# fims9000/SYNT_ISIC

Measured on AMD Instinct MI355X. Metric: images/sec at 3x64x64 T=1000 (DDPM reverse-diffusion sampling), higher is better.
Workload: dtype f32

## Files before the change

synt_isic_amd/csrc/common.h:

```cpp
#pragma once

#include <hip/hip_runtime.h>

#include <atomic>
#include <cstdarg>
#include <cstdint>
#include <cstdio>
#include <string>
#include <map>
#include <mutex>
#include <vector>

#include "../../include/sisic.h"

namespace sisic {

void set_error(const char* fmt, ...);

#define SISIC_HIP(call)                                                                   \
    do {                                                                                  \
        hipError_t _e = (call);                                                           \
        if (_e != hipSuccess) {                                                           \
            ::sisic::set_error("%s failed: %s (%s:%d)", #call, hipGetErrorString(_e),     \
                               __FILE__, __LINE__);                                       \
            return SISIC_EHIP;                                                            \
        }                                                                                 \
    } while (0)

#define SISIC_REQUIRE(cond, ...)                 \
    do {                                         \
        if (!(cond)) {                           \
            ::sisic::set_error(__VA_ARGS__);     \
            return SISIC_EINVAL;                 \
        }                                        \
    } while (0)

#define SISIC_TRY(expr)             \
    do {                            \
        int _rc = (expr);           \
        if (_rc != SISIC_OK) return _rc; \
    } while (0)

enum ProfileKind { PK_CONV3 = 0, PK_CONV1 = 1, PK_GN = 2, PK_ATTN = 3, PK_DDPM = 4, PK_OTHER = 5, PK_WINO_MAIN = 6, PK_WINO_BF3 = 7, PK_COUNT = 8 };

struct ProfileSlot {
    double ms = 0, bytes = 0, flops = 0, flops_exec = 0;
    int64_t launches = 0;
};

struct PendingEvent {
    hipEvent_t start, stop;
    int kind;
    int kind2;
};

}

struct sisic_ctx {
    int device = 0;
    int num_cus = 0;
    bool profiling = false;
    sisic::ProfileSlot prof[sisic::PK_COUNT];
    std::vector<sisic::PendingEvent> pending;
    std::vector<hipEvent_t> event_pool;
    struct SplitK { float* p = nullptr; size_t floats = 0; };
    std::map<hipStream_t, SplitK> splitk;
    std::mutex splitk_mutex;
    std::atomic<uint64_t> scratch_generation{0};
};

namespace sisic {

struct ProfileScope {
    sisic_ctx* ctx;
    hipStream_t stream;
    PendingEvent ev{};
    bool active = false;
    ProfileScope(sisic_ctx* c, hipStream_t s, int kind, double bytes, double flops, double flops_exec = -1.0, int kind2 = -1);
    ~ProfileScope();
};

int profile_collect(sisic_ctx* ctx);

inline int ensure_dynamic_lds(sisic_ctx* ctx, const void* kern, int bytes, std::atomic<uint64_t>& done) {
    const uint64_t bit = uint64_t(1) << (ctx->device & 63);
    if (done.load(std::memory_order_acquire) & bit) return SISIC_OK;
    SISIC_HIP(hipFuncSetAttribute(kern, hipFuncAttributeMaxDynamicSharedMemorySize, bytes));
    done.fetch_or(bit, std::memory_order_release);
    return SISIC_OK;
}

inline int cdiv(int a, int b) { return (a + b - 1) / b; }
inline int wino_latency_ksplit(int Cout, int Cin, int Hout, int Wout) {
    const int co_t = Cout > 64 ? 128 : 64;
    const int per_image = cdiv(Hout, 8) * cdiv(Wout, 16) * cdiv(Cout, co_t);
    const int nchunks = cdiv(Cin, 8);
    int k = 1;
    while (per_image * k < 256 && k < 8 && nchunks % (2 * k) == 0) k *= 2;
    return k;
}
inline int wino_latency_segments(int Hout, int Wout) { return cdiv(Hout * Wout, 1024); }
inline int64_t cdiv64(int64_t a, int64_t b) { return (a + b - 1) / b; }
inline int round_up(int a, int b) { return cdiv(a, b) * b; }

constexpr int CONV_CO_TILE = 64;
inline int conv_ci_chunk(int ksize) { return ksize == 1 ? 32 : (ksize == 3 ? 16 : 4); }
inline int conv_cin_pad(int cin, int ksize) { return round_up(cin, conv_ci_chunk(ksize)); }
inline int conv_cout_pad(int cout) { return round_up(cout, CONV_CO_TILE); }
inline int64_t conv_packed_floats(int cout, int cin, int ksize) {
    const int64_t first = (int64_t)conv_cin_pad(cin, ksize) * ksize * ksize * conv_cout_pad(cout);
    return ksize == 1 ? 3 * first + first / 2 : first;
}

int launch_conv2d(sisic_ctx*, const sisic_conv_args& a, hipStream_t s);
int launch_conv_smallcout(sisic_ctx*, const sisic_conv_args& a, hipStream_t s);
int launch_score_head_bwd(sisic_ctx*, const float* logits, const float* fc_w, const float* act, float* g, int B, int C,
                          int HW, int n_classes, int target, hipStream_t s);
int launch_relu_bwd(sisic_ctx*, const float* dy, const float* y, float* out, int64_t n, hipStream_t s);
int launch_scatter_add_even(sisic_ctx*, float* dst, const float* src, int planes, int H, int W, hipStream_t s);
int launch_maxpool_bwd(sisic_ctx*, const float* dm, const float* xin, float* dx, int planes, int H, int W, hipStream_t s);
int launch_stem_bwd(sisic_ctx*, const float* g, const float* w_oihw, float* dp, int B, int CO, int OH, int OW, int H, int W,
                    hipStream_t s);
int launch_preprocess_bwd(sisic_ctx*, const float* dp, const float* x, float* dx, int B, int H, int W, int OH, int OW,
                          hipStream_t s);
int launch_add_relu(sisic_ctx*, const float* y, const float* identity, float* out, int64_t n, hipStream_t s);
int launch_gradcam(sisic_ctx*, const float* y, const float* outp, const float* fc_w, const float* bias, float* cam, int B, int C,
                   int h, int w, int S, int target, hipStream_t s);
int conv_stats_slots(const sisic_conv_args& a);
bool conv_finalizes(const sisic_conv_args& a);
bool conv_pointwise_applicable(const sisic_conv_args& a);
int conv_pointwise_stats_slots(const sisic_conv_args& a);
int launch_conv_pointwise(sisic_ctx*, const sisic_conv_args& a, hipStream_t s);
bool conv_pointwise_bf3_applicable(const sisic_conv_args& a);
int launch_conv_pointwise_bf3(sisic_ctx*, const sisic_conv_args& a, hipStream_t s);
int launch_gn_finalize(sisic_ctx*, const float* st0, int c0, int slots0, const float* st1, int c1, int slots1, int B,
                       int HW, int groups, float eps, const float* gamma, const float* beta, float* scale, float* shift,
                       hipStream_t s, float* mean_rstd = nullptr);
int launch_conv_winograd(sisic_ctx*, const sisic_conv_args& a, const float* u_packed, int cfg, hipStream_t s);
int launch_winograd_pack(sisic_ctx*, const float* w, int Cout, int Cin, float* packed, hipStream_t s);
int64_t winograd_packed_numel(int Cout, int Cin);
inline int64_t winograd_first_floats(int Cout, int Cin) { return (int64_t)round_up(Cin, 16) * 16 * conv_cout_pad(Cout); }
int launch_conv_pack(sisic_ctx*, const float* w, int Cout, int Cin, int k, float* packed, hipStream_t s);
int launch_gn_stats(sisic_ctx*, const float* in0, int c0, const float* in1, int c1, int B, int HW, int groups,
                    float eps, const float* gamma, const float* beta, float* scale, float* shift, hipStream_t s,
                    float* mean_rstd = nullptr);
int launch_attention(sisic_ctx*, const float* qkv, float* out, int B, int C, int N, int head_dim, hipStream_t s);
int launch_ddpm_step(sisic_ctx*, const float* eps, const float* x, const float* z, float* out, int64_t n,
                     float sb, float sa, float c0, float c1, float sigma, float clip, hipStream_t s);
size_t loop_state_bytes();
int launch_loop_select_row(sisic_ctx*, const float* table, int R, const void* state, float* out, hipStream_t s);
int launch_loop_advance(sisic_ctx*, void* state, hipStream_t s);
int launch_ddpm_step_indexed(sisic_ctx*, const float* eps, float* x, int64_t n, const void* state, const float* coef,
                             const int* zrow, float clip, hipStream_t s);
int launch_denorm_u8(sisic_ctx*, const float* x, uint8_t* out, int B, int C, int H, int W, hipStream_t s, int form = 0);
int launch_temb_mlp(sisic_ctx*, const float* t_vals, int B, const float* freqs, int n_freqs, const float* w1t,
                    const float* b1, const float* w2t, const float* b2, int hidden, float* temb_act, hipStream_t s,
                    float* save_emb = nullptr, float* save_h1 = nullptr, float* save_t2 = nullptr);
int launch_linear_t(sisic_ctx*, const float* x, int B, int K, const float* wt, const float* bias, int R,
                    float* out, hipStream_t s);
int launch_transpose2d(sisic_ctx*, const float* in, int rows, int cols, float* out, int out_ld, int out_col0,
                       hipStream_t s);
int launch_preprocess(sisic_ctx*, const float* x, float* out, int B, int H, int W, int OH, int OW, hipStream_t s);
int launch_maxpool(sisic_ctx*, const float* x, float* out, int B, int C, int H, int W, hipStream_t s);
int launch_avgpool_fc(sisic_ctx*, const float* x, const float* w, const float* bias, float* out, int B, int C, int HW,
                      int n_out, hipStream_t s);
int launch_class_scores(sisic_ctx*, const float* logits, int B, int n, int target, float* prob, float* logscore,
                        hipStream_t s);
int launch_mask_patches(sisic_ctx*, const float* image, const uint8_t* masks, float* out, int S, int C, int H, int W,
                        int patch, hipStream_t s);

}
```

synt_isic_amd/csrc/conv_mfma.hip:

```cpp
#include <cstdlib>
#include <type_traits>

#include "common.h"
#include "pack_device.h"

namespace sisic {

typedef float f32x16 __attribute__((ext_vector_type(16)));

struct ConvParams {
    const float* in0;
    const float* in1;
    int c0, c1;
    int B, Hin, Win;
    int Hc, Wc;
    int Hout, Wout;
    int ups;
    int zero_insert;
    const float* w;
    int cout_pad;
    const float* bias;
    int Cout;
    const float* gn_scale;
    const float* gn_shift;
// ... 108 lines not shown
    const int a_base = half * G::KK * G::CO_TILE + wm * MT * 32 + l31;
    int b_base;
    {
        const int pix = wn * NT * 32 + l31;
        const int y = pix / TW, x = pix % TW;
        b_base = half * G::CHS + (y * STRIDE) * G::IW + x * STRIDE;
    }
    constexpr int NT_STEP = (TW >= 32) ? ((TW > 32) ? 32 * STRIDE : STRIDE * G::IW) : (32 / TW) * STRIDE * G::IW;
    static_assert(TW >= 32 || 32 % TW == 0, "TW must divide 32");
    static_assert(TW <= 32 || TW % 32 == 0, "TW must be a multiple of 32");

    f32x16 acc[MT][NT];
#pragma unroll
    for (int m = 0; m < MT; ++m)
#pragma unroll
        for (int n = 0; n < NT; ++n)
#pragma unroll
            for (int r = 0; r < 16; ++r) acc[m][n][r] = 0.0f;

    float rin[G::EPT];
    float rw[G::W_F4_PT * 4];
    float gsc = 1.0f, gsh = 0.0f;
    bool cval = false;

    const int prologue = (p.gn_scale == nullptr) ? 0 : (p.gn_silu ? 2 : 1);

    auto load_chunk = [&](int chunk) __attribute__((always_inline)) {
        const int c = chunk * CIC + sci;
        cval = c < Cin;
        const int cc = min(c, Cin - 1);
        const float* src = (cc < p.c0) ? p.in0 + ((size_t)b * p.c0 + cc) * HWin
                                       : p.in1 + ((size_t)b * p.c1 + (cc - p.c0)) * HWin;
        if constexpr (V4) {
#pragma unroll
            for (int i = 0; i < EPT4; ++i) {
                const float4 t = *reinterpret_cast<const float4*>(src + goff4[i]);
                rin[4 * i + 0] = t.x; rin[4 * i + 1] = t.y; rin[4 * i + 2] = t.z; rin[4 * i + 3] = t.w;
            }
        } else {
#pragma unroll
            for (int i = 0; i < G::EPT; ++i) rin[i] = src[goff[i]];
        }
        if (prologue) {
            gsc = p.gn_scale[(size_t)b * Cin + cc];
            gsh = p.gn_shift[(size_t)b * Cin + cc];
        }
        const float* wsrc = p.w + (size_t)chunk * CIC * G::KK * p.cout_pad + co0;
#pragma unroll
        for (int i = 0; i < G::W_F4_PT; ++i) {
            const int f = min(tid + i * G::NTHR, G::W_F4 - 1);
            const int rr = f / (G::CO_TILE / 4), c4 = f % (G::CO_TILE / 4);
            const float4 t = *reinterpret_cast<const float4*>(wsrc + (size_t)rr * p.cout_pad + c4 * 4);
            rw[4 * i + 0] = t.x; rw[4 * i + 1] = t.y; rw[4 * i + 2] = t.z; rw[4 * i + 3] = t.w;
        }
    };

    auto store_chunk = [&](const int buf) __attribute__((always_inline)) {
        float* dst = in_lds + buf * G::IN_BUF + sci * G::CHS + sl;
        const unsigned m = cval ? vmask : 0u;
        float v[G::EPT];
        if (prologue == 2) {
#pragma unroll
            for (int i = 0; i < G::EPT; ++i) v[i] = silu_f(rin[i] * gsc + gsh);
        } else if (prologue == 1) {
#pragma unroll
            for (int i = 0; i < G::EPT; ++i) v[i] = rin[i] * gsc + gsh;
        } else {
#pragma unroll
            for (int i = 0; i < G::EPT; ++i) v[i] = rin[i];
        }
        if constexpr (V4) {
            float* dst4 = in_lds + buf * G::IN_BUF + sci * G::CHS + 4 * sl;
            const unsigned m4 = cval ? vmask4 : 0u;
#pragma unroll
            for (int i = 0; i < EPT4; ++i) {
                const bool on = (m4 >> i) & 1u;
                *reinterpret_cast<float4*>(dst4 + i * G::TPC * 4) =
                    make_float4(on ? v[4 * i + 0] : 0.0f, on ? v[4 * i + 1] : 0.0f, on ? v[4 * i + 2] : 0.0f, on ? v[4 * i + 3] : 0.0f);
            }
        } else {
#pragma unroll
            for (int i = 0; i < G::EPT; ++i) dst[i * G::TPC] = ((m >> i) & 1u) ? v[i] : 0.0f;
        }
        float* wdst = w_lds + buf * G::W_BUF + tid * 4;
#pragma unroll
        for (int i = 0; i < G::W_F4_PT; ++i)
            *reinterpret_cast<float4*>(wdst + i * G::NTHR * 4) =
                make_float4(rw[4 * i + 0], rw[4 * i + 1], rw[4 * i + 2], rw[4 * i + 3]);
    };

    auto compute_chunk = [&](const int buf) __attribute__((always_inline)) {
        const float* A = w_lds + buf * G::W_BUF + a_base;
        const float* Bm = in_lds + buf * G::IN_BUF + b_base;
#pragma unroll
        for (int cp = kg * (CIC / 2 / KSP); cp < (kg + 1) * (CIC / 2 / KSP); ++cp) {
#pragma unroll
            for (int ky = 0; ky < KS; ++ky) {
#pragma unroll
                for (int kx = 0; kx < KS; ++kx) {
                    float a[MT], bb[NT];
#pragma unroll
                    for (int m = 0; m < MT; ++m)
                        a[m] = A[(2 * cp * G::KK + ky * KS + kx) * G::CO_TILE + m * 32];
#pragma unroll
                    for (int n = 0; n < NT; ++n)
                        bb[n] = Bm[2 * cp * G::CHS + ky * G::IW + kx + n * NT_STEP];
#pragma unroll
                    for (int m = 0; m < MT; ++m)
#pragma unroll
                        for (int n = 0; n < NT; ++n)
                            acc[m][n] = __builtin_amdgcn_mfma_f32_32x32x2f32(a[m], bb[n], acc[m][n], 0, 0, 0);
                }
            }
        }
    };

    load_chunk(0);
    store_chunk(0);
    __syncthreads();
    auto step = [&](const int chunk, auto buf_tag) __attribute__((always_inline)) {
        constexpr int BUF = decltype(buf_tag)::value;
        const bool more = chunk + 1 < p.nchunks;
        if (more) load_chunk(chunk + 1);
        compute_chunk(BUF);
        if (more) store_chunk(BUF ^ 1);
        __syncthreads();
    };
    {
        int chunk = 0;
        for (; chunk + 1 < p.nchunks; chunk += 2) {
            step(chunk, std::integral_constant<int, 0>{});
            step(chunk + 1, std::integral_constant<int, 1>{});
        }
        if (chunk < p.nchunks) step(chunk, std::integral_constant<int, 0>{});
    }

    if constexpr (KSP > 1) {
        static_assert(KSP == 2, "two K groups");
        static_assert((size_t)WM * WN * MT * NT * 16 * 64 * sizeof(float) <= G::LDS_BYTES, "reduction slab fits the staging LDS");
        float* red = smem + (size_t)wq * MT * NT * 16 * 64 + lane;
        if (kg == 1) {
#pragma unroll
            for (int m = 0; m < MT; ++m)
#pragma unroll
                for (int n = 0; n < NT; ++n)
#pragma unroll
                    for (int r = 0; r < 16; ++r) red[((m * NT + n) * 16 + r) * 64] = acc[m][n][r];
        }
        __syncthreads();
        if (kg != 0) return;
#pragma unroll
        for (int m = 0; m < MT; ++m)
#pragma unroll
            for (int n = 0; n < NT; ++n)
#pragma unroll
                for (int r = 0; r < 16; ++r) acc[m][n][r] += red[((m * NT + n) * 16 + r) * 64];
    }

    const size_t HWout = (size_t)p.Hout * p.Wout;
    float cbias[MT][16];
#pragma unroll
    for (int m = 0; m < MT; ++m) {
#pragma unroll
        for (int r = 0; r < 16; ++r) {
            cbias[m][r] = 0.0f;
        }
    }
    if (p.bias) {
#pragma unroll
        for (int m = 0; m < MT; ++m)
#pragma unroll
            for (int r = 0; r < 16; ++r)
                cbias[m][r] += p.bias[min(co0 + wm * MT * 32 + m * 32 + (r & 3) + 8 * (r >> 2) + 4 * half, p.Cout - 1)];
    }
    if (p.chan_bias) {
        const float* cb = p.chan_bias + (size_t)b * p.chan_bias_stride;
#pragma unroll
        for (int m = 0; m < MT; ++m)
#pragma unroll
            for (int r = 0; r < 16; ++r)
                cbias[m][r] += cb[min(co0 + wm * MT * 32 + m * 32 + (r & 3) + 8 * (r >> 2) + 4 * half, p.Cout - 1)];
    }
    float psum[MT][16];
#pragma unroll
    for (int m = 0; m < MT; ++m)
#pragma unroll
        for (int r = 0; r < 16; ++r) psum[m][r] = 0.0f;
    unsigned pvmask = 0;
#pragma unroll
    for (int n = 0; n < NT; ++n) {
        const int pix = wn * NT * 32 + n * 32 + l31;
        const int oy = oy0 + pix / TW, ox = ox0 + pix % TW;
        const bool pv = oy < p.Hout && ox < p.Wout;
        pvmask |= pv ? (1u << n) : 0u;
        const size_t pix_off = (size_t)min(oy, p.Hout - 1) * p.Wout + min(ox, p.Wout - 1);
#pragma unroll
        for (int m = 0; m < MT; ++m) {
            float res[16];
#pragma unroll
            for (int r = 0; r < 16; ++r) res[r] = 0.0f;
            if (p.residual) {
#pragma unroll
                for (int r = 0; r < 16; ++r) {
                    const int co = min(co0 + wm * MT * 32 + m * 32 + (r & 3) + 8 * (r >> 2) + 4 * half, p.Cout - 1);
                    res[r] = p.residual[((size_t)b * p.Cout + co) * HWout + pix_off];
                }
            }
#pragma unroll
            for (int r = 0; r < 16; ++r) {
                const int co = co0 + wm * MT * 32 + m * 32 + (r & 3) + 8 * (r >> 2) + 4 * half;
                float v = acc[m][n][r] + cbias[m][r] + res[r];
                if (p.relu) v = fmaxf(v, 0.0f);
                if (pv && co < p.Cout) p.out[((size_t)b * p.Cout + co) * HWout + pix_off] = v;
                acc[m][n][r] = v;
                psum[m][r] += pv ? v : 0.0f;
            }
        }
    }

    if (p.stats) {
        const float cnt = half_wave_sum((float)__builtin_popcount(pvmask));
        const float inv = 1.0f / fmaxf(cnt, 1.0f);
        const int slots = p.tiles_x * p.tiles_y * WN, slot = (ty * p.tiles_x + tx) * WN + wn;
#pragma unroll
        for (int m = 0; m < MT; ++m) {
#pragma unroll
            for (int r = 0; r < 16; ++r) {
                const int co = co0 + wm * MT * 32 + m * 32 + (r & 3) + 8 * (r >> 2) + 4 * half;
                const float s1 = half_wave_sum(psum[m][r]);
                const float mean = s1 * inv;
                float q = 0.0f;
#pragma unroll
                for (int n = 0; n < NT; ++n) {
                    const float d = acc[m][n][r] - mean;
                    q += ((pvmask >> n) & 1u) ? d * d : 0.0f;
                }
                q = half_wave_sum(q);
                if (l31 == 0 && co < p.Cout)
                    reinterpret_cast<float4*>(p.stats)[((size_t)b * p.Cout + co) * slots + slot] = make_float4(cnt, s1, q, 0.0f);
            }
        }
    }
}


__global__ void conv_pack_kernel(const float* __restrict__ w, int Cout, int Cin, int KK, int cin_pad, int cout_pad,
                                 float* __restrict__ out) {
    const size_t first = (size_t)cin_pad * KK * cout_pad;
    const size_t total = KK == 1 ? 3 * first + first / 2 : first;
    for (size_t i = (size_t)blockIdx.x * blockDim.x + threadIdx.x; i < total; i += (size_t)gridDim.x * blockDim.x) {
        conv_pack_elem(i, w, Cout, Cin, KK, cin_pad, cout_pad, out);
    }
}

template <int KS, int STRIDE, int MT, int NT, int WM, int WN, int TW, int CIC, int OCC = 2, int KSP = 1>
static int launch_cfg(sisic_ctx* ctx, ConvParams& p, hipStream_t s) {
    using G = ConvGeom<KS, STRIDE, MT, NT, WM, WN, TW, CIC, KSP>;
    p.tiles_x = cdiv(p.Wout, TW);
    p.tiles_y = cdiv(p.Hout, G::TH);
    p.n_co_tiles = p.cout_pad / G::CO_TILE;
    p.nchunks = cdiv(p.c0 + p.c1, CIC);
    const int64_t nwg = (int64_t)p.B * p.tiles_x * p.tiles_y * p.n_co_tiles;
    SISIC_REQUIRE(nwg > 0 && nwg < (int64_t(1) << 31), "conv2d: grid of %lld workgroups unsupported", (long long)nwg);
    p.nwg = (int)nwg;
    if (p.slots_query) {
        *p.slots_query = p.tiles_x * p.tiles_y * WN;
        return SISIC_OK;
    }
    if constexpr (KS == 1 && STRIDE == 1 && TW == G::PIX && G::EPT % 4 == 0) {
        const bool aligned = ((reinterpret_cast<uintptr_t>(p.in0) | reinterpret_cast<uintptr_t>(p.in1)) & 15) == 0;
        if (p.Wc % 4 == 0 && aligned) {
            auto kern4 = conv_mfma_kernel<KS, STRIDE, MT, NT, WM, WN, TW, CIC, OCC, KSP, true>;
            static std::atomic<uint64_t> lds_opt_in4{0};
            SISIC_TRY(ensure_dynamic_lds(ctx, reinterpret_cast<const void*>(kern4), (int)G::LDS_BYTES, lds_opt_in4));
            hipLaunchKernelGGL(kern4, dim3(p.nwg), dim3(G::NTHR), G::LDS_BYTES, s, p);
            SISIC_HIP(hipGetLastError());
            return SISIC_OK;
        }
    }
    auto kern = conv_mfma_kernel<KS, STRIDE, MT, NT, WM, WN, TW, CIC, OCC, KSP>;
    static std::atomic<uint64_t> lds_opt_in{0};
    SISIC_TRY(ensure_dynamic_lds(ctx, reinterpret_cast<const void*>(kern), (int)G::LDS_BYTES, lds_opt_in));
    hipLaunchKernelGGL(kern, dim3(p.nwg), dim3(G::NTHR), G::LDS_BYTES, s, p);
    SISIC_HIP(hipGetLastError());
    return SISIC_OK;
}

int launch_conv_pack(sisic_ctx*, const float* w, int Cout, int Cin, int k, float* packed, hipStream_t s) {
    SISIC_REQUIRE(k == 1 || k == 3 || k == 7, "conv_pack: ksize %d unsupported", k);
    const int cin_pad = conv_cin_pad(Cin, k), cout_pad = conv_cout_pad(Cout);
    const size_t total = (size_t)cin_pad * k * k * cout_pad;
    const int blocks = (int)std::min<size_t>((total * (k == 1 ? 4 : 1) + 255) / 256, 4096);
    hipLaunchKernelGGL(conv_pack_kernel, dim3(blocks), dim3(256), 0, s, w, Cout, Cin, k * k, cin_pad, cout_pad, packed);
    SISIC_HIP(hipGetLastError());
    return SISIC_OK;
}

static int dispatch_conv2d(sisic_ctx* ctx, const sisic_conv_args& a, hipStream_t s, int* slots_query);

static int winograd_cfg(const sisic_conv_args& a) {
    if (!(a.ksize == 3 && a.stride == 1 && a.w_winograd != nullptr && a.Cout > 4) || a.upsample == 2) return 0;
    if ((a.tile_cfg >= 60 && a.tile_cfg <= 74) || a.tile_cfg == 78 || a.tile_cfg == 79 || (a.tile_cfg >= 90 && a.tile_cfg <= 92)) return a.tile_cfg;
    if (a.tile_cfg != 0) return 0;
    const int Hout = a.Hin << (a.upsample ? 1 : 0), Wout = a.Win << (a.upsample ? 1 : 0);
    const bool fits32 = 16.0 * std::max(a.c0, a.c1) * a.Hin * a.Win < 4294967296.0;
    if (!fits32) return 0;
    if (Hout >= 12 && Wout >= 12) {
        static const bool wide_on = [] { const char* e = std::getenv("SISIC_WINO_WIDE"); return !e || std::atoi(e) != 0; }();
        static const bool bf3_on = [] { const char* e = std::getenv("SISIC_WINO_BF16X3"); return !e || std::atoi(e) != 0; }();
        const int th = (Hout + 15) / 16 * 16, tw = (Wout + 15) / 16 * 16;
        if (bf3_on && a.Cout % 64 == 0 && 4 * Hout * Wout >= 3 * th * tw && a.c0 + a.c1 >= 16 &&
            a.c0 + a.c1 <= 2048 &&
            4.0 * a.Cout * Hout * Wout < 2147483648.0)
            return 74;
        if (wide_on && !a.upsample) return a.Cout > 64 ? 68 : 69;
        return 66;
    }
    const int Cin = a.c0 + a.c1;
    static const bool ksplit_on = [] { const char* e = std::getenv("SISIC_KSPLIT"); return !e || std::atoi(e) != 0; }();
    if (ksplit_on && Hout <= 8 && Wout <= 8 && Hout >= 5 && Wout >= 5 && Cin >= 128 && Cin % 32 == 0 && a.Cout >= 128) {
        static const bool wide_on = [] { const char* e = std::getenv("SISIC_WINO_WIDE"); return !e || std::atoi(e) != 0; }();
        static const bool bf3_on = [] { const char* e = std::getenv("SISIC_WINO_BF16X3"); return !e || std::atoi(e) != 0; }();
        if (bf3_on && !a.upsample && a.Cout % 64 == 0 && Cin <= 512) return 92;
        return (wide_on && !a.upsample) ? 91 : 90;
    }
    return 0;
}
static bool winograd_selected(const sisic_conv_args& a) { return winograd_cfg(a) != 0; }

int conv_stats_slots(const sisic_conv_args& a) {
    if (const int cfg = winograd_cfg(a)) {
        if (cfg >= 90 && cfg <= 92) return 1;
        const int Hout = a.Hin << (a.upsample ? 1 : 0), Wout = a.Win << (a.upsample ? 1 : 0);
        if ((cfg == 78 || cfg == 79) && wino_latency_ksplit(a.Cout, a.c0 + a.c1, Hout, Wout) > 1) return wino_latency_segments(Hout, Wout);
        if ((cfg >= 68 && cfg <= 73) || cfg == 78 || cfg == 79) return ((Hout + 7) / 8) * ((Wout + 15) / 16);
        const int edge = (cfg == 61 || cfg == 63 || cfg == 65 || cfg == 67) ? 8 : 16;
        return ((Hout + edge - 1) / edge) * ((Wout + edge - 1) / edge);
    }
    int slots = 0;
    sisic_conv_args q = a;
    q.stats_out = nullptr;
    if (dispatch_conv2d(nullptr, q, nullptr, &slots) != SISIC_OK) return 0;
    return slots;
}

bool conv_finalizes(const sisic_conv_args& a) {
    if (!a.fin_gamma || a.fin_groups <= 0) return false;
    const int cfg = winograd_cfg(a);
    const int Hout = a.Hin << (a.upsample ? 1 : 0), Wout = a.Win << (a.upsample ? 1 : 0);
    if (a.Cout % a.fin_groups != 0 || a.Cout / a.fin_groups != 8) return false;
    if (cfg == 74) return !a.upsample && Hout <= 16 && Wout <= 16 && a.Cout % 64 == 0;
    if (cfg < 90 || cfg > 92) return false;
    if (Hout * Wout != 64 || a.Cout % 16 != 0) return false;
    return ((reinterpret_cast<uintptr_t>(a.residual) | reinterpret_cast<uintptr_t>(a.out) | reinterpret_cast<uintptr_t>(a.stats_out)) & 15) == 0;
}

int launch_conv2d(sisic_ctx* ctx, const sisic_conv_args& a, hipStream_t s) { return dispatch_conv2d(ctx, a, s, nullptr); }

static int dispatch_conv2d(sisic_ctx* ctx, const sisic_conv_args& a, hipStream_t s, int* slots_query) {
    SISIC_REQUIRE(a.in0 && a.w_packed && a.out, "conv2d: null tensor");
    SISIC_REQUIRE(a.B > 0 && a.Hin > 0 && a.Win > 0 && a.c0 > 0 && a.c1 >= 0 && a.Cout > 0, "conv2d: bad shape");
    SISIC_REQUIRE((a.c1 == 0) == (a.in1 == nullptr), "conv2d: in1/c1 mismatch");
    SISIC_REQUIRE(a.ksize == 1 || a.ksize == 3 || a.ksize == 7, "conv2d: ksize %d unsupported", a.ksize);
    SISIC_REQUIRE(a.stride == 1 || a.stride == 2, "conv2d: stride %d unsupported", a.stride);
    SISIC_REQUIRE(a.ksize != 7 || a.stride == 2, "conv2d: 7x7 is built for stride 2 only (the ResNet stem)");
    SISIC_REQUIRE(!(a.upsample && a.stride != 1), "conv2d: upsample with stride");
    SISIC_REQUIRE((a.gn_scale == nullptr) == (a.gn_shift == nullptr), "conv2d: gn_scale/gn_shift mismatch");

    ConvParams p{};
    p.in0 = a.in0; p.in1 = a.in1; p.c0 = a.c0; p.c1 = a.c1;
    p.B = a.B; p.Hin = a.Hin; p.Win = a.Win;
    p.ups = a.upsample ? 1 : 0;
    p.zero_insert = a.upsample == 2 ? 1 : 0;
    p.Hc = a.Hin << p.ups; p.Wc = a.Win << p.ups;
    const int pad = a.ksize / 2;
    p.Hout = (p.Hc + 2 * pad - a.ksize) / a.stride + 1;
    p.Wout = (p.Wc + 2 * pad - a.ksize) / a.stride + 1;
    p.w = a.w_packed; p.cout_pad = conv_cout_pad(a.Cout);
    p.bias = a.bias; p.Cout = a.Cout;
    p.gn_scale = a.gn_scale; p.gn_shift = a.gn_shift; p.gn_silu = a.gn_silu;
    p.chan_bias = a.chan_bias; p.chan_bias_stride = a.chan_bias_stride; p.residual = a.residual; p.relu = a.relu; p.out = a.out;
    p.stats = a.stats_out; p.slots_query = slots_query;

    const int Cin = a.c0 + a.c1;
    const double kk = double(a.ksize) * a.ksize;
    const double out_elems = double(a.B) * a.Cout * p.Hout * p.Wout;
    const double bytes = 4.0 * (double(a.B) * Cin * a.Hin * a.Win + out_elems) + 4.0 * (Cin * a.Cout * kk + a.Cout) +
                         (a.residual ? 4.0 * out_elems : 0.0);
    const double flops = 2.0 * out_elems * Cin * kk;
    int cfg = a.tile_cfg;
    const bool use_wino = winograd_selected(a);
    SISIC_REQUIRE(a.stats_out == nullptr || conv_stats_slots(a) > 0,
                  "conv2d: stats_out given but sisic_conv_stats_slots() is 0 for these arguments");
    const bool wino_ups9 = use_wino && a.upsample && !a.gn_scale && winograd_cfg(a) == 66;
    ProfileScope prof(slots_query ? nullptr : ctx, s, a.ksize == 1 ? PK_CONV1 : PK_CONV3, bytes, flops,
                      use_wino ? flops * (wino_ups9 ? 9.0 : 16.0) / 36.0 : flops,
                      (use_wino && winograd_cfg(a) == 74) ? PK_WINO_BF3 :
                      (use_wino && !wino_ups9 && (winograd_cfg(a) == 66 || (winograd_cfg(a) >= 68 && winograd_cfg(a) <= 73) || winograd_cfg(a) == 78 || winograd_cfg(a) == 79)) ? PK_WINO_MAIN : -1);

    if (a.ksize == 3 && a.stride == 1 && !a.upsample && a.Cout <= 4 && (cfg == 0 || (cfg >= 50 && cfg <= 52))) {
        if (slots_query) return SISIC_OK;
        return launch_conv_smallcout(ctx, a, s);
    }
    if (use_wino) {
        SISIC_REQUIRE(!slots_query, "conv2d: internal: slot query on the Winograd path");
        return launch_conv_winograd(ctx, a, a.w_winograd, winograd_cfg(a), s);
    }
    SISIC_REQUIRE((cfg < 60 || cfg > 74) && cfg != 78 && cfg != 79 && (cfg < 90 || cfg > 92), "conv2d: tile_cfg %d needs w_winograd, ksize 3 and stride 1", cfg);
    if (a.ksize == 7) {
        if (cfg == 0) cfg = 41;
        if (cfg == 41) return launch_cfg<7, 2, 2, 1, 1, 4, 32, 2>(ctx, p, s);
        if (cfg == 42) return launch_cfg<7, 2, 2, 1, 1, 4, 32, 4>(ctx, p, s);
    } else if (a.ksize == 1 && a.stride == 2) {
        if (cfg == 0) cfg = p.Wout >= 24 ? 31 : (p.Wout >= 12 ? 32 : 33);
        switch (cfg) {
            case 31: return launch_cfg<1, 2, 2, 1, 1, 4, 32, 16>(ctx, p, s);
            case 32: return launch_cfg<1, 2, 2, 1, 1, 4, 16, 16>(ctx, p, s);
            case 33: return launch_cfg<1, 2, 1, 1, 2, 2, 8, 16>(ctx, p, s);
        }
    } else if (a.ksize == 1) {
        p.Hin = 1; p.Win = a.Hin * a.Win; p.Hc = 1; p.Wc = p.Win; p.Hout = 1; p.Wout = p.Win; p.ups = 0;
        SISIC_REQUIRE(!a.upsample, "conv2d: 1x1 with upsample");
        static const bool pw_on = [] { const char* e = std::getenv("SISIC_POINTWISE"); return !e || std::atoi(e) != 0; }();
        static const bool pwb_on = [] { const char* e = std::getenv("SISIC_POINTWISE_BF16X3"); return !e || std::atoi(e) != 0; }();
        if ((cfg == 0 && pwb_on && conv_pointwise_bf3_applicable(a)) || (cfg >= 28 && cfg <= 30) || cfg == 34 || cfg == 35) {
            if (slots_query) { *slots_query = conv_pointwise_stats_slots(a); return SISIC_OK; }
            return launch_conv_pointwise_bf3(ctx, a, s);
        }
        if ((cfg == 0 && pw_on && conv_pointwise_applicable(a)) || cfg == 20) {
            if (slots_query) { *slots_query = conv_pointwise_stats_slots(a); return SISIC_OK; }
            return launch_conv_pointwise(ctx, a, s);
        }
        if (cfg == 0) cfg = (p.Wout <= 64) ? 22 : (p.Wout <= 256 ? 25 : 24);
        switch (cfg) {
            case 21: return launch_cfg<1, 1, 2, 2, 1, 4, 256, 16>(ctx, p, s);
            case 22: return launch_cfg<1, 1, 1, 1, 2, 2, 64, 16>(ctx, p, s);
            case 23: return launch_cfg<1, 1, 2, 1, 1, 4, 128, 16>(ctx, p, s);
            case 24: return launch_cfg<1, 1, 1, 2, 2, 4, 256, 32, 4>(ctx, p, s);
            case 25: return launch_cfg<1, 1, 1, 1, 2, 4, 128, 32, 4>(ctx, p, s);
            case 26: return launch_cfg<1, 1, 1, 2, 2, 4, 256, 16, 4>(ctx, p, s);
            case 27: return launch_cfg<1, 1, 1, 1, 2, 4, 128, 16, 4>(ctx, p, s);
        }
    } else if (a.stride == 1) {
        if (cfg == 0) cfg = p.Wout >= 24 ? 8 : (p.Wout >= 12 ? 9 : 16);
        switch (cfg) {
            case 1: return launch_cfg<3, 1, 2, 2, 1, 4, 64, 8>(ctx, p, s);
            case 2: return launch_cfg<3, 1, 2, 2, 1, 4, 32, 8>(ctx, p, s);
            case 3: return launch_cfg<3, 1, 2, 2, 1, 4, 16, 8>(ctx, p, s);
            case 4: return launch_cfg<3, 1, 1, 1, 2, 2, 8, 8>(ctx, p, s);
            case 16: return launch_cfg<3, 1, 1, 1, 2, 2, 8, 16, 2, 2>(ctx, p, s);
            case 17: return launch_cfg<3, 1, 1, 1, 2, 2, 8, 8, 2, 2>(ctx, p, s);
            case 5: return launch_cfg<3, 1, 2, 1, 1, 4, 16, 8>(ctx, p, s);
            case 6: return launch_cfg<3, 1, 2, 1, 1, 4, 64, 8>(ctx, p, s);
            case 7: return launch_cfg<3, 1, 2, 1, 1, 4, 32, 8>(ctx, p, s);
            case 8: return launch_cfg<3, 1, 1, 2, 2, 4, 32, 8, 4>(ctx, p, s);
            case 9: return launch_cfg<3, 1, 1, 2, 2, 4, 16, 8, 4>(ctx, p, s);
            case 10: return launch_cfg<3, 1, 1, 2, 2, 4, 32, 8, 2>(ctx, p, s);
            case 14: return launch_cfg<3, 1, 1, 1, 2, 4, 16, 8, 4>(ctx, p, s);
            case 15: return launch_cfg<3, 1, 1, 1, 2, 4, 8, 8, 4>(ctx, p, s);
        }
    } else {
        if (cfg == 0) cfg = p.Wout >= 24 ? 11 : (p.Wout >= 12 ? 12 : 18);
        switch (cfg) {
            case 11: return launch_cfg<3, 2, 2, 1, 1, 4, 32, 8>(ctx, p, s);
            case 12: return launch_cfg<3, 2, 2, 1, 1, 4, 16, 8>(ctx, p, s);
            case 13: return launch_cfg<3, 2, 1, 1, 2, 2, 8, 8>(ctx, p, s);
            case 18: return launch_cfg<3, 2, 1, 1, 2, 2, 8, 16, 2, 2>(ctx, p, s);
            case 19: return launch_cfg<3, 2, 1, 1, 2, 2, 8, 8, 2, 2>(ctx, p, s);
        }
    }
    set_error("conv2d: tile_cfg %d invalid for ksize %d stride %d", cfg, a.ksize, a.stride);
    return SISIC_EINVAL;
}

}
```

synt_isic_amd/csrc/conv_small.hip:

```cpp
#include <atomic>
#include <type_traits>

#include "common.h"

namespace sisic {

constexpr int CS_TW = 32, CS_PX = 4, CS_CIC = 2;
constexpr int CS_IW = CS_TW + 2;
constexpr int CS_IWP = 36;
template <int CS_TH>
struct CSGeom;
template <int CS_TH, int KS>
constexpr size_t cs_lds_bytes();
template <int CS_TH>
struct CSGeom {
    static constexpr int THR = (CS_TW / CS_PX) * CS_TH;
    static constexpr int IH = CS_TH + 2;
    static constexpr int TPC = THR / CS_CIC;
    static constexpr int EPT = (IH * CS_IWP + TPC - 1) / TPC;
    static constexpr int CHS = EPT * TPC;
    static_assert(CS_IWP >= CS_IW + 2 && CS_IWP % 4 == 0 && CHS % 4 == 0, "aligned rows");
    static_assert(CS_CIC * 9 <= THR, "one thread per filter row");
};

template <int CS_TH, int KS>
constexpr size_t cs_lds_bytes() {
    constexpr size_t in = (size_t)KS * 2 * CS_CIC * CSGeom<CS_TH>::CHS, red = (size_t)(KS - 1) * CS_PX * 4 * CSGeom<CS_TH>::THR;
    return sizeof(float) * (in > red ? in : red);
}

struct ConvSmallParams {
    const float* in0;
    const float* in1;
    int c0, c1, B, H, W;
    const float* w;
    int cout_pad;
    const float* bias;
    int Cout;
    const float* gn_scale;
    const float* gn_shift;
    int gn_silu;
    const float* chan_bias;
    int chan_bias_stride;
    const float* residual;
    int relu;
    float* out;
    int tiles_x, tiles_y, nchunks;
};

template <int CS_TH, int KS>
__global__ void __launch_bounds__(CSGeom<CS_TH>::THR * KS, KS == 1 ? 3 : 4) conv3x3_smallcout_kernel(const ConvSmallParams p) {
    constexpr int CS_THR = CSGeom<CS_TH>::THR, CS_IH = CSGeom<CS_TH>::IH, CS_TPC = CSGeom<CS_TH>::TPC, CS_EPT = CSGeom<CS_TH>::EPT,
                  CS_CHS = CSGeom<CS_TH>::CHS;
    constexpr int IN_FLOATS = 2 * CS_CIC * CS_CHS, RED_FLOATS = (KS - 1) * CS_PX * 4 * CS_THR;
    extern __shared__ __attribute__((aligned(16))) float lds_all[];
    __shared__ __attribute__((aligned(16))) float w_all[KS][2][CS_CIC * 9 * 4];
    const int grp = KS == 1 ? 0 : __builtin_amdgcn_readfirstlane((int)threadIdx.x / CS_THR);
    float (*in_lds)[CS_CIC * CS_CHS] = reinterpret_cast<float (*)[CS_CIC * CS_CHS]>(lds_all + grp * IN_FLOATS);
    float (*w_lds)[CS_CIC * 9 * 4] = w_all[grp];

    int tile = blockIdx.x;
    const int tx = tile % p.tiles_x;
    tile /= p.tiles_x;
    const int ty = tile % p.tiles_y;
    const int b = tile / p.tiles_y;
    const int oy0 = ty * CS_TH, ox0 = tx * CS_TW;
    const int tid = threadIdx.x - grp * CS_THR;
    const int sci = tid / CS_TPC, sl = tid % CS_TPC;
    const int HW = p.H * p.W, Cin = p.c0 + p.c1;
    const int prologue = (p.gn_scale == nullptr) ? 0 : (p.gn_silu ? 2 : 1);
    const int n_mine = p.nchunks / KS, c_first = grp * n_mine;

    int goff[CS_EPT];
    unsigned vmask = 0;
#pragma unroll
    for (int i = 0; i < CS_EPT; ++i) {
        const int e = sl + i * CS_TPC;
        const int yy = e / CS_IWP, xx = e % CS_IWP;
        const int gy = oy0 - 1 + yy, gx = ox0 - 1 + xx;
        const bool v = yy < CS_IH && xx < CS_IW && gy >= 0 && gy < p.H && gx >= 0 && gx < p.W;
        goff[i] = v ? gy * p.W + gx : 0;
        vmask |= (v ? 1u : 0u) << i;
    }

    float rin[CS_EPT];
    float rw[4];
    float gsc = 1.0f, gsh = 0.0f;
    bool cval = false;

    auto load_chunk = [&](int chunk) {
        const int c = chunk * CS_CIC + sci;
        cval = c < Cin;
        const int cc = min(c, Cin - 1);
        const float* src = (cc < p.c0) ? p.in0 + ((size_t)b * p.c0 + cc) * HW : p.in1 + ((size_t)b * p.c1 + (cc - p.c0)) * HW;
#pragma unroll
        for (int i = 0; i < CS_EPT; ++i) rin[i] = src[goff[i]];
        if (prologue) {
            gsc = p.gn_scale[(size_t)b * Cin + cc];
            gsh = p.gn_shift[(size_t)b * Cin + cc];
        }
        const int row = min(tid, CS_CIC * 9 - 1);
        const float4 t = *reinterpret_cast<const float4*>(p.w + ((size_t)chunk * CS_CIC * 9 + row) * p.cout_pad);
        rw[0] = t.x; rw[1] = t.y; rw[2] = t.z; rw[3] = t.w;
    };
    auto store_chunk = [&](int buf) {
        float* dst = &in_lds[buf][sci * CS_CHS + sl];
        const unsigned m = cval ? vmask : 0u;
#pragma unroll
        for (int i = 0; i < CS_EPT; ++i) {
            float v = rin[i];
            if (prologue) v = v * gsc + gsh;
            if (prologue == 2) v = v * __builtin_amdgcn_rcpf(1.0f + __expf(-v));
            dst[i * CS_TPC] = ((m >> i) & 1u) ? v : 0.0f;
        }
        if (tid < CS_CIC * 9) *reinterpret_cast<float4*>(&w_lds[buf][tid * 4]) = make_float4(rw[0], rw[1], rw[2], rw[3]);
    };

    const int py = tid / (CS_TW / CS_PX), px0 = (tid % (CS_TW / CS_PX)) * CS_PX;
    float acc[CS_PX][4];
#pragma unroll
    for (int q = 0; q < CS_PX; ++q)
#pragma unroll
        for (int co = 0; co < 4; ++co) acc[q][co] = 0.0f;
    load_chunk(c_first);
    store_chunk(0);
    __syncthreads();
    for (int k = 0; k < n_mine; ++k) {
        const int chunk = c_first + k;
        const int buf = k & 1;
        const bool more = k + 1 < n_mine;
        if (more) load_chunk(chunk + 1);
        const float* I = &in_lds[buf][py * CS_IWP + px0];
        const float* Wt = &w_lds[buf][0];
#pragma unroll 1
        for (int ci = 0; ci < CS_CIC; ++ci) {
#pragma unroll
            for (int ky = 0; ky < 3; ++ky) {
                const float* row = I + ci * CS_CHS + ky * CS_IWP;
                const float4 r4 = *reinterpret_cast<const float4*>(row);
                const float2 r2 = *reinterpret_cast<const float2*>(row + 4);
                const float in[6] = {r4.x, r4.y, r4.z, r4.w, r2.x, r2.y};
#pragma unroll
                for (int kx = 0; kx < 3; ++kx) {
                    const float4 w4 = *reinterpret_cast<const float4*>(&Wt[(ci * 9 + ky * 3 + kx) * 4]);
#pragma unroll
                    for (int q = 0; q < CS_PX; ++q) {
                        const float a = in[q + kx];
                        acc[q][0] += a * w4.x; acc[q][1] += a * w4.y; acc[q][2] += a * w4.z; acc[q][3] += a * w4.w;
                    }
                }
            }
        }
        if (more) store_chunk(buf ^ 1);
        __syncthreads();
    }
    if constexpr (KS > 1) {
        if (grp > 0) {
#pragma unroll
            for (int q = 0; q < CS_PX; ++q)
#pragma unroll
                for (int co = 0; co < 4; ++co) lds_all[((grp - 1) * CS_PX * 4 + q * 4 + co) * CS_THR + tid] = acc[q][co];
        }
        __syncthreads();
        if (grp > 0) return;
#pragma unroll
        for (int g = 1; g < KS; ++g)
#pragma unroll
            for (int q = 0; q < CS_PX; ++q)
#pragma unroll
                for (int co = 0; co < 4; ++co) acc[q][co] += lds_all[((g - 1) * CS_PX * 4 + q * 4 + co) * CS_THR + tid];
    }

    const int oy = oy0 + py, ox = ox0 + px0;
    if (oy < p.H) {
        const bool vec = (p.W & 3) == 0;
#pragma unroll
        for (int co = 0; co < 4; ++co) {
            if (co < p.Cout) {
                const size_t base = ((size_t)b * p.Cout + co) * HW + (size_t)oy * p.W;
                float add = 0.0f;
                if (p.bias) add += p.bias[co];
                if (p.chan_bias) add += p.chan_bias[(size_t)b * p.chan_bias_stride + co];
                float v[CS_PX];
#pragma unroll
                for (int q = 0; q < CS_PX; ++q) {
                    v[q] = acc[q][co] + add;
                    if (p.residual && ox + q < p.W) v[q] += p.residual[base + ox + q];
                    if (p.relu) v[q] = fmaxf(v[q], 0.0f);
                }
                if (vec) {
                    if (ox < p.W) *reinterpret_cast<float4*>(p.out + base + ox) = make_float4(v[0], v[1], v[2], v[3]);
                } else {
#pragma unroll
                    for (int q = 0; q < CS_PX; ++q)
                        if (ox + q < p.W) p.out[base + ox + q] = v[q];
                }
            }
        }
    }
}

int launch_conv_smallcout(sisic_ctx* ctx, const sisic_conv_args& a, hipStream_t s) {
    ConvSmallParams p{};
    p.in0 = a.in0; p.in1 = a.in1; p.c0 = a.c0; p.c1 = a.c1; p.B = a.B; p.H = a.Hin; p.W = a.Win;
    p.w = a.w_packed; p.cout_pad = conv_cout_pad(a.Cout); p.bias = a.bias; p.Cout = a.Cout;
    p.gn_scale = a.gn_scale; p.gn_shift = a.gn_shift; p.gn_silu = a.gn_silu;
    p.chan_bias = a.chan_bias; p.chan_bias_stride = a.chan_bias_stride; p.residual = a.residual; p.relu = a.relu;
    p.out = a.out;
    p.tiles_x = cdiv(a.Win, CS_TW);
    p.nchunks = cdiv(a.c0 + a.c1, CS_CIC);
    const bool spare = a.tile_cfg == 50 || (a.tile_cfg != 51 && (int64_t)a.B * p.tiles_x * cdiv(a.Hin, 32) >= 256);
    p.tiles_y = cdiv(a.Hin, spare ? 32 : 8);
    const int64_t nwg = (int64_t)a.B * p.tiles_x * p.tiles_y;
    SISIC_REQUIRE(nwg > 0 && nwg < (int64_t(1) << 31), "conv2d(small): grid too large");
    const bool ksplit = a.tile_cfg != 52 && p.nchunks % 4 == 0 && p.nchunks >= 16;
    auto go = [&](auto th_tag, auto ks_tag) -> int {
        constexpr int TH = decltype(th_tag)::value, KSV = decltype(ks_tag)::value;
        auto kern = conv3x3_smallcout_kernel<TH, KSV>;
        static std::atomic<uint64_t> opt{0};
        SISIC_TRY(ensure_dynamic_lds(ctx, reinterpret_cast<const void*>(kern), (int)(cs_lds_bytes<TH, KSV>()), opt));
        constexpr size_t lds = cs_lds_bytes<TH, KSV>();
        constexpr unsigned thr = (unsigned)(CSGeom<TH>::THR * KSV);
        hipLaunchKernelGGL(kern, dim3((unsigned)nwg), dim3(thr), lds, s, p);
        return SISIC_OK;
    };
    using I = std::integral_constant<int, 1>;
    if (ksplit) {
        if (spare) SISIC_TRY(go(std::integral_constant<int, 32>{}, std::integral_constant<int, 4>{}));
        else SISIC_TRY(go(std::integral_constant<int, 8>{}, std::integral_constant<int, 4>{}));
    } else {
        if (spare) SISIC_TRY(go(std::integral_constant<int, 32>{}, I{}));
        else SISIC_TRY(go(std::integral_constant<int, 8>{}, I{}));
    }
    SISIC_HIP(hipGetLastError());
    return SISIC_OK;
}

}
```

Measured before the change: 11.82.

## Add streaming direct conv for few-input-channel 3x3 convs and wider smallcout tiles

Adds a new direct 3x3 convolution kernel for convs with at most 4 input channels (such as the UNet stem on 3-channel images). It stages a strip of rows in LDS, computes 8 output channels by 4 pixels per thread, and emits per-slot GroupNorm statistics with DPP reductions. This path is taken instead of Winograd or MFMA for these shapes. The small-Cout output conv also gets a 64x16 tile variant when the width is a multiple of 64. Both are enabled by default through the SISIC_EDGE_FORMS environment variable, and they change tiling and the stats slot layout for these layers.

```diff
diff --git a/synt_isic_amd/csrc/common.h b/synt_isic_amd/csrc/common.h
--- a/synt_isic_amd/csrc/common.h
+++ b/synt_isic_amd/csrc/common.h
@@ -114,6 +114,9 @@
 
 int launch_conv2d(sisic_ctx*, const sisic_conv_args& a, hipStream_t s);
 int launch_conv_smallcout(sisic_ctx*, const sisic_conv_args& a, hipStream_t s);
+bool conv_stream_applicable(const sisic_conv_args& a);
+int conv_stream_stats_slots(const sisic_conv_args& a);
+int launch_conv_stream(sisic_ctx*, const sisic_conv_args& a, hipStream_t s);
 int launch_score_head_bwd(sisic_ctx*, const float* logits, const float* fc_w, const float* act, float* g, int B, int C,
                           int HW, int n_classes, int target, hipStream_t s);
 int launch_relu_bwd(sisic_ctx*, const float* dy, const float* y, float* out, int64_t n, hipStream_t s);
diff --git a/synt_isic_amd/csrc/conv_mfma.hip b/synt_isic_amd/csrc/conv_mfma.hip
--- a/synt_isic_amd/csrc/conv_mfma.hip
+++ b/synt_isic_amd/csrc/conv_mfma.hip
@@ -434,6 +434,7 @@
     if (!(a.ksize == 3 && a.stride == 1 && a.w_winograd != nullptr && a.Cout > 4) || a.upsample == 2) return 0;
     if ((a.tile_cfg >= 60 && a.tile_cfg <= 74) || a.tile_cfg == 78 || a.tile_cfg == 79 || (a.tile_cfg >= 90 && a.tile_cfg <= 92)) return a.tile_cfg;
     if (a.tile_cfg != 0) return 0;
+    if (conv_stream_applicable(a)) return 0;
     const int Hout = a.Hin << (a.upsample ? 1 : 0), Wout = a.Win << (a.upsample ? 1 : 0);
     const bool fits32 = 16.0 * std::max(a.c0, a.c1) * a.Hin * a.Win < 4294967296.0;
     if (!fits32) return 0;
@@ -530,7 +531,11 @@
                       (use_wino && winograd_cfg(a) == 74) ? PK_WINO_BF3 :
                       (use_wino && !wino_ups9 && (winograd_cfg(a) == 66 || (winograd_cfg(a) >= 68 && winograd_cfg(a) <= 73) || winograd_cfg(a) == 78 || winograd_cfg(a) == 79)) ? PK_WINO_MAIN : -1);
 
-    if (a.ksize == 3 && a.stride == 1 && !a.upsample && a.Cout <= 4 && (cfg == 0 || (cfg >= 50 && cfg <= 52))) {
+    if (cfg == 56 || (cfg == 0 && conv_stream_applicable(a))) {
+        if (slots_query) { *slots_query = conv_stream_stats_slots(a); return SISIC_OK; }
+        return launch_conv_stream(ctx, a, s);
+    }
+    if (a.ksize == 3 && a.stride == 1 && !a.upsample && a.Cout <= 4 && (cfg == 0 || (cfg >= 50 && cfg <= 53))) {
         if (slots_query) return SISIC_OK;
         return launch_conv_smallcout(ctx, a, s);
     }
diff --git a/synt_isic_amd/csrc/conv_small.hip b/synt_isic_amd/csrc/conv_small.hip
--- a/synt_isic_amd/csrc/conv_small.hip
+++ b/synt_isic_amd/csrc/conv_small.hip
@@ -1,31 +1,28 @@
 #include <atomic>
+#include <cstdlib>
 #include <type_traits>
 
 #include "common.h"
 
 namespace sisic {
 
-constexpr int CS_TW = 32, CS_PX = 4, CS_CIC = 2;
-constexpr int CS_IW = CS_TW + 2;
-constexpr int CS_IWP = 36;
-template <int CS_TH>
-struct CSGeom;
-template <int CS_TH, int KS>
-constexpr size_t cs_lds_bytes();
-template <int CS_TH>
+constexpr int CS_PX = 4, CS_CIC = 2;
+template <int CS_TW, int CS_TH>
 struct CSGeom {
+    static constexpr int IW = CS_TW + 2;
+    static constexpr int IWP = CS_TW + 4;
     static constexpr int THR = (CS_TW / CS_PX) * CS_TH;
     static constexpr int IH = CS_TH + 2;
     static constexpr int TPC = THR / CS_CIC;
-    static constexpr int EPT = (IH * CS_IWP + TPC - 1) / TPC;
+    static constexpr int EPT = (IH * IWP + TPC - 1) / TPC;
     static constexpr int CHS = EPT * TPC;
-    static_assert(CS_IWP >= CS_IW + 2 && CS_IWP % 4 == 0 && CHS % 4 == 0, "aligned rows");
+    static_assert(IWP >= IW + 2 && IWP % 4 == 0 && CHS % 4 == 0, "aligned rows");
     static_assert(CS_CIC * 9 <= THR, "one thread per filter row");
 };
 
-template <int CS_TH, int KS>
+template <int CS_TW, int CS_TH, int KS>
 constexpr size_t cs_lds_bytes() {
-    constexpr size_t in = (size_t)KS * 2 * CS_CIC * CSGeom<CS_TH>::CHS, red = (size_t)(KS - 1) * CS_PX * 4 * CSGeom<CS_TH>::THR;
+    constexpr size_t in = (size_t)KS * 2 * CS_CIC * CSGeom<CS_TW, CS_TH>::CHS, red = (size_t)(KS - 1) * CS_PX * 4 * CSGeom<CS_TW, CS_TH>::THR;
     return sizeof(float) * (in > red ? in : red);
 }
 
@@ -48,10 +45,10 @@
     int tiles_x, tiles_y, nchunks;
 };
 
-template <int CS_TH, int KS>
-__global__ void __launch_bounds__(CSGeom<CS_TH>::THR * KS, KS == 1 ? 3 : 4) conv3x3_smallcout_kernel(const ConvSmallParams p) {
-    constexpr int CS_THR = CSGeom<CS_TH>::THR, CS_IH = CSGeom<CS_TH>::IH, CS_TPC = CSGeom<CS_TH>::TPC, CS_EPT = CSGeom<CS_TH>::EPT,
-                  CS_CHS = CSGeom<CS_TH>::CHS;
+template <int CS_TW, int CS_TH, int KS>
+__global__ void __launch_bounds__((CSGeom<CS_TW, CS_TH>::THR * KS), (KS == 1 ? 3 : 4)) conv3x3_smallcout_kernel(const ConvSmallParams p) {
+    using G = CSGeom<CS_TW, CS_TH>;
+    constexpr int CS_THR = G::THR, CS_IH = G::IH, CS_TPC = G::TPC, CS_EPT = G::EPT, CS_CHS = G::CHS, CS_IW = G::IW, CS_IWP = G::IWP;
     constexpr int IN_FLOATS = 2 * CS_CIC * CS_CHS, RED_FLOATS = (KS - 1) * CS_PX * 4 * CS_THR;
     extern __shared__ __attribute__((aligned(16))) float lds_all[];
     __shared__ __attribute__((aligned(16))) float w_all[KS][2][CS_CIC * 9 * 4];
@@ -207,31 +204,37 @@
     p.gn_scale = a.gn_scale; p.gn_shift = a.gn_shift; p.gn_silu = a.gn_silu;
     p.chan_bias = a.chan_bias; p.chan_bias_stride = a.chan_bias_stride; p.residual = a.residual; p.relu = a.relu;
     p.out = a.out;
-    p.tiles_x = cdiv(a.Win, CS_TW);
     p.nchunks = cdiv(a.c0 + a.c1, CS_CIC);
-    const bool spare = a.tile_cfg == 50 || (a.tile_cfg != 51 && (int64_t)a.B * p.tiles_x * cdiv(a.Hin, 32) >= 256);
-    p.tiles_y = cdiv(a.Hin, spare ? 32 : 8);
+    static const bool edge_on = [] { const char* e = std::getenv("SISIC_EDGE_FORMS"); return !e || std::atoi(e) != 0; }();
+    const bool spare = a.tile_cfg == 50 || a.tile_cfg == 53 ||
+                       (a.tile_cfg != 51 && (int64_t)a.B * cdiv(a.Win, 32) * cdiv(a.Hin, 32) >= 256);
+    const bool wide = a.tile_cfg == 53 || (a.tile_cfg == 0 && edge_on && spare && a.Win % 64 == 0);
+    const int tw = wide ? 64 : 32, th = wide ? 16 : (spare ? 32 : 8);
+    p.tiles_x = cdiv(a.Win, tw);
+    p.tiles_y = cdiv(a.Hin, th);
     const int64_t nwg = (int64_t)a.B * p.tiles_x * p.tiles_y;
     SISIC_REQUIRE(nwg > 0 && nwg < (int64_t(1) << 31), "conv2d(small): grid too large");
     const bool ksplit = a.tile_cfg != 52 && p.nchunks % 4 == 0 && p.nchunks >= 16;
-    auto go = [&](auto th_tag, auto ks_tag) -> int {
-        constexpr int TH = decltype(th_tag)::value, KSV = decltype(ks_tag)::value;
-        auto kern = conv3x3_smallcout_kernel<TH, KSV>;
+    auto go = [&](auto tw_tag, auto th_tag, auto ks_tag) -> int {
+        constexpr int TW = decltype(tw_tag)::value, TH = decltype(th_tag)::value, KSV = decltype(ks_tag)::value;
+        auto kern = conv3x3_smallcout_kernel<TW, TH, KSV>;
         static std::atomic<uint64_t> opt{0};
-        SISIC_TRY(ensure_dynamic_lds(ctx, reinterpret_cast<const void*>(kern), (int)(cs_lds_bytes<TH, KSV>()), opt));
-        constexpr size_t lds = cs_lds_bytes<TH, KSV>();
-        constexpr unsigned thr = (unsigned)(CSGeom<TH>::THR * KSV);
+        constexpr size_t lds = cs_lds_bytes<TW, TH, KSV>();
+        SISIC_TRY(ensure_dynamic_lds(ctx, reinterpret_cast<const void*>(kern), (int)lds, opt));
+        constexpr unsigned thr = (unsigned)(CSGeom<TW, TH>::THR * KSV);
         hipLaunchKernelGGL(kern, dim3((unsigned)nwg), dim3(thr), lds, s, p);
         return SISIC_OK;
     };
-    using I = std::integral_constant<int, 1>;
-    if (ksplit) {
-        if (spare) SISIC_TRY(go(std::integral_constant<int, 32>{}, std::integral_constant<int, 4>{}));
-        else SISIC_TRY(go(std::integral_constant<int, 8>{}, std::integral_constant<int, 4>{}));
-    } else {
-        if (spare) SISIC_TRY(go(std::integral_constant<int, 32>{}, I{}));
-        else SISIC_TRY(go(std::integral_constant<int, 8>{}, I{}));
-    }
+    using C8 = std::integral_constant<int, 8>;
+    using C16 = std::integral_constant<int, 16>;
+    using C32 = std::integral_constant<int, 32>;
+    using C64 = std::integral_constant<int, 64>;
+    auto go_ks = [&](auto ks_tag) -> int {
+        if (wide) return go(C64{}, C16{}, ks_tag);
+        return spare ? go(C32{}, C32{}, ks_tag) : go(C32{}, C8{}, ks_tag);
+    };
+    if (ksplit) SISIC_TRY(go_ks(std::integral_constant<int, 4>{}));
+    else SISIC_TRY(go_ks(std::integral_constant<int, 1>{}));
     SISIC_HIP(hipGetLastError());
     return SISIC_OK;
 }
diff --git a/synt_isic_amd/csrc/conv_stream.hip b/synt_isic_amd/csrc/conv_stream.hip
--- /dev/null
+++ b/synt_isic_amd/csrc/conv_stream.hip
@@ -0,0 +1,143 @@
+#include <cstdlib>
+
+#include "common.h"
+
+namespace sisic {
+
+constexpr int CST_THR = 256, CST_PXW = 128, CST_CO = 64, CST_MAXCIN = 4;
+constexpr int CST_IN_FLOATS = 1600;
+
+struct ConvStreamParams {
+    const float* in;
+    int Cin, H, W;
+    const float* w;
+    int cout_pad;
+    const float* bias;
+    int Cout;
+    const float* chan_bias;
+    int chan_bias_stride;
+    float* out;
+    float* stats;
+    int rows, slots;
+};
+
+__device__ __forceinline__ float cst_half_wave_sum(float v) {
+    v += __int_as_float(__builtin_amdgcn_update_dpp(0, __float_as_int(v), 0xB1, 0xf, 0xf, true));
+    v += __int_as_float(__builtin_amdgcn_update_dpp(0, __float_as_int(v), 0x4E, 0xf, 0xf, true));
+    v += __int_as_float(__builtin_amdgcn_update_dpp(0, __float_as_int(v), 0x141, 0xf, 0xf, true));
+    v += __int_as_float(__builtin_amdgcn_update_dpp(0, __float_as_int(v), 0x140, 0xf, 0xf, true));
+    return v + __shfl_xor(v, 16);
+}
+
+__global__ void __launch_bounds__(CST_THR) conv_stream_kernel(const ConvStreamParams p) {
+    __shared__ __attribute__((aligned(16))) float in_l[CST_IN_FLOATS];
+    __shared__ __attribute__((aligned(16))) float w_l[CST_MAXCIN * 9 * CST_CO];
+    const int tid = threadIdx.x;
+    const int seg = blockIdx.x % p.slots, b = blockIdx.x / p.slots;
+    const int R = p.rows, W = p.W, H = p.H, Cin = p.Cin;
+    const int WP = W + 4, RP = R + 2;
+    const int y0 = seg * R;
+    const int HW = H * W;
+
+    const float* src = p.in + (size_t)b * Cin * HW;
+    for (int e = tid; e < Cin * RP * WP; e += CST_THR) {
+        const int xx = e % WP, r = e / WP;
+        const int yy = r % RP, ci = r / RP;
+        const int gy = y0 - 1 + yy, gx = xx - 1;
+        in_l[e] = (gy >= 0 && gy < H && gx >= 0 && gx < W) ? src[(size_t)ci * HW + gy * W + gx] : 0.0f;
+    }
+
+    const int q = tid & 31, cg = tid >> 5;
+    const int P = min(R, H - y0) * W;
+    const bool active = 4 * q < P;
+    const int ly = active ? (4 * q) / W : 0, x = active ? (4 * q) % W : 0;
+    const float cnt = (float)P;
+
+    for (int co0 = 0; co0 < p.Cout; co0 += CST_CO) {
+        if (co0 > 0) __syncthreads();
+        for (int e = tid; e < Cin * 9 * CST_CO; e += CST_THR) {
+            const int co = co0 + e % CST_CO, r = e / CST_CO;
+            w_l[e] = co < p.Cout ? p.w[(size_t)r * p.cout_pad + co] : 0.0f;
+        }
+        __syncthreads();
+        const int cb = co0 + 8 * cg;
+        if (cb >= p.Cout) continue;
+
+        float acc[8][4];
+#pragma unroll
+        for (int j = 0; j < 8; ++j)
+#pragma unroll
+            for (int k = 0; k < 4; ++k) acc[j][k] = 0.0f;
+        for (int ci = 0; ci < Cin; ++ci) {
+#pragma unroll
+            for (int ky = 0; ky < 3; ++ky) {
+                const float* row = in_l + (ci * RP + ly + ky) * WP + x;
+                const float4 r4 = *reinterpret_cast<const float4*>(row);
+                const float2 r2 = *reinterpret_cast<const float2*>(row + 4);
+                const float v[6] = {r4.x, r4.y, r4.z, r4.w, r2.x, r2.y};
+#pragma unroll
+                for (int kx = 0; kx < 3; ++kx) {
+                    const float* wr = w_l + (ci * 9 + ky * 3 + kx) * CST_CO + 8 * cg;
+                    const float4 wa = *reinterpret_cast<const float4*>(wr);
+                    const float4 wb = *reinterpret_cast<const float4*>(wr + 4);
+                    const float wv[8] = {wa.x, wa.y, wa.z, wa.w, wb.x, wb.y, wb.z, wb.w};
+#pragma unroll
+                    for (int j = 0; j < 8; ++j)
+#pragma unroll
+                        for (int k = 0; k < 4; ++k) acc[j][k] = __builtin_fmaf(v[k + kx], wv[j], acc[j][k]);
+                }
+            }
+        }
+
+#pragma unroll
+        for (int j = 0; j < 8; ++j) {
+            const int co = cb + j;
+            float add = 0.0f;
+            if (p.bias) add += p.bias[co];
+            if (p.chan_bias) add += p.chan_bias[(size_t)b * p.chan_bias_stride + co];
+            const float4 o = make_float4(acc[j][0] + add, acc[j][1] + add, acc[j][2] + add, acc[j][3] + add);
+            const size_t plane = ((size_t)b * p.Cout + co) * HW;
+            if (active) *reinterpret_cast<float4*>(p.out + plane + (size_t)(y0 + ly) * W + x) = o;
+            if (p.stats) {
+                const float s1 = cst_half_wave_sum(active ? (o.x + o.y) + (o.z + o.w) : 0.0f);
+                const float mean = s1 / cnt;
+                const float d0 = o.x - mean, d1 = o.y - mean, d2 = o.z - mean, d3 = o.w - mean;
+                const float m2 = cst_half_wave_sum(active ? (d0 * d0 + d1 * d1) + (d2 * d2 + d3 * d3) : 0.0f);
+                if (q == 0) reinterpret_cast<float4*>(p.stats)[((size_t)b * p.Cout + co) * p.slots + seg] = make_float4(cnt, s1, m2, 0.0f);
+            }
+        }
+    }
+}
+
+static int stream_rows(int W) { return CST_PXW / W; }
+
+bool conv_stream_applicable(const sisic_conv_args& a) {
+    static const bool edge_on = [] { const char* e = std::getenv("SISIC_EDGE_FORMS"); return !e || std::atoi(e) != 0; }();
+    if (!(a.tile_cfg == 56 || (a.tile_cfg == 0 && edge_on))) return false;
+    return a.ksize == 3 && a.stride == 1 && !a.upsample && a.in1 == nullptr && a.c1 == 0 && a.c0 <= CST_MAXCIN &&
+           a.gn_scale == nullptr && a.residual == nullptr && !a.relu && a.Cout > 4 && a.Cout % 8 == 0 && a.Win % 4 == 0 &&
+           a.Win <= CST_PXW;
+}
+
+int conv_stream_stats_slots(const sisic_conv_args& a) { return cdiv(a.Hin, stream_rows(a.Win)); }
+
+int launch_conv_stream(sisic_ctx*, const sisic_conv_args& a, hipStream_t s) {
+    SISIC_REQUIRE(conv_stream_applicable(a), "conv2d: tile_cfg 56 needs a plain 3x3 stride-1 convolution of <= 4 input channels, "
+                                             "Cout %% 8 == 0 and a width that is a multiple of 4 up to 128");
+    ConvStreamParams p{};
+    p.in = a.in0; p.Cin = a.c0; p.H = a.Hin; p.W = a.Win;
+    p.w = a.w_packed; p.cout_pad = conv_cout_pad(a.Cout); p.bias = a.bias; p.Cout = a.Cout;
+    p.chan_bias = a.chan_bias; p.chan_bias_stride = a.chan_bias_stride; p.out = a.out; p.stats = a.stats_out;
+    p.rows = stream_rows(a.Win);
+    p.slots = conv_stream_stats_slots(a);
+    SISIC_REQUIRE(a.c0 * (p.rows + 2) * (a.Win + 4) <= CST_IN_FLOATS, "conv2d(stream): internal: input table too small");
+    static_assert(CST_MAXCIN * (CST_PXW / 4 + 2) * (4 + 4) <= CST_IN_FLOATS && CST_MAXCIN * 3 * (CST_PXW + 4) <= CST_IN_FLOATS,
+                  "input table covers both ends of the width range");
+    const int64_t nwg = (int64_t)a.B * p.slots;
+    SISIC_REQUIRE(nwg > 0 && nwg < (int64_t(1) << 31), "conv2d(stream): grid too large");
+    hipLaunchKernelGGL(conv_stream_kernel, dim3((unsigned)nwg), dim3(CST_THR), 0, s, p);
+    SISIC_HIP(hipGetLastError());
+    return SISIC_OK;
+}
+
+}
```

Measured after the change: 11.83, median of 6. No clear change (+0.0%).
